# SonyCSLParis/audio-metrics

Hardware: AMD Instinct MI355X
Metric: evaluate() embeddings/sec (FAD+KD+PRDC), 2×100k CLAP-512 sets, 1/2/4/8 GPUs (higher is better)
Workload: dtype f32

## Files before the change

### audio-metrics_amd/_lib.py

```python
import ctypes
import os
from ctypes import c_char_p, c_double, c_int, c_int64, c_size_t, c_void_p

from ._build import DEV_LIB_PATH, LIB_PATH

_P = c_void_p

SIGNATURES = {
    "am_version": (c_char_p, []),
    "am_status_string": (c_char_p, [c_int]),
    "am_last_error": (c_char_p, []),
    "am_stats_workspace_bytes": (c_size_t, [c_int64, c_int]),
    "am_stats_f32": (c_int, [_P, c_int64, c_int, c_int64, _P, _P, _P, c_size_t, _P]),
    "am_colsum_f32": (c_int, [_P, c_int64, c_int, c_int64, _P, _P, c_size_t, _P]),
    "am_scatter_f32": (c_int, [_P, c_int64, c_int, c_int64, _P, _P, _P, c_size_t, _P]),
    "am_stats_f64_workspace_bytes": (c_size_t, [c_int64, c_int]),
    "am_stats_f64": (c_int, [_P, c_int64, c_int, c_int64, _P, _P, _P, c_size_t, _P]),
    "am_colsum_f64": (c_int, [_P, c_int64, c_int, c_int64, _P, _P, c_size_t, _P]),
    "am_scatter_f64": (c_int, [_P, c_int64, c_int, c_int64, _P, _P, _P, c_size_t, _P]),
    "am_stats_gather_workspace_bytes": (c_size_t, [c_int64, c_int, c_int]),
    "am_stats_gather_f32": (c_int, [_P, c_int64, c_int64, c_int, _P, _P, c_int, _P, _P, _P, c_size_t, _P]),
    "am_stats_gather_f64": (c_int, [_P, c_int64, c_int64, c_int, _P, _P, c_int, _P, _P, _P, c_size_t, _P]),
    "am_stats_merge_f64": (c_int, [c_int64, _P, _P, c_int64, _P, _P, c_int, _P, _P, _P]),
    "am_stats_push_max_rows": (c_int, []),
    "am_stats_push_f32": (c_int, [_P, c_int64, c_int, c_int64, c_int64, _P, _P, _P, _P, c_int64, _P]),
    "am_frechet_workspace_bytes": (c_size_t, [c_int]),
    "am_frechet_f64": (c_int, [_P, _P, _P, _P, c_int, c_int, c_double, _P, _P, c_size_t, _P]),
    "am_frechet_first_block": (c_int, []),
    "am_frechet_enqueue_f64": (c_int, [_P, _P, _P, _P, c_int, c_int, c_int, c_int, c_double, _P, _P, c_size_t, _P]),
    "am_frechet_batch_workspace_bytes": (c_size_t, [c_int, c_int]),
    "am_frechet_batch_f64": (c_int, [_P, _P, _P, _P, c_int64, c_int, c_int, c_int, c_double, _P, _P, c_size_t, _P]),
    "am_frechet_groups_max_rows": (c_int, []),
    "am_frechet_groups_workspace_bytes": (c_size_t, [c_int64, c_int, c_int]),
    "am_frechet_groups_f32": (c_int, [_P, c_int64, c_int64, c_int, _P, _P, c_int, _P, _P, _P, _P, c_size_t, _P]),
    "am_frechet_groups_f64": (c_int, [_P, c_int64, c_int64, c_int, _P, _P, c_int, _P, _P, _P, _P, c_size_t, _P]),
    "am_apa_f64": (c_double, [c_double, c_double, c_double]),
    "am_kd_workspace_bytes": (c_size_t, [c_int, c_int]),
    "am_kd_poly_workspace_bytes": (c_size_t, [c_int, c_int, c_int]),
    "am_kd_poly_f32": (c_int, [_P, c_int64, c_int64, _P, c_int64, c_int64, c_int, _P, _P, c_int, c_int,
                               c_double, c_double, c_int, _P, _P, c_size_t, _P]),
    "am_kd_draw_indices": (c_int, [ctypes.c_uint64, ctypes.c_uint64, ctypes.c_uint64, ctypes.c_uint64, c_int64, c_int64, c_int,
                                   c_int, _P, _P]),
    "am_kd_rbf_workspace_bytes": (c_size_t, [c_int, c_int]),
    "am_kd_rbf_f32": (c_int, [_P, c_int64, c_int64, _P, c_int64, c_int64, c_int, _P, _P, c_int, c_int, c_double, _P, _P,
                              c_size_t, _P]),
    "am_pairwise_select_workspace_bytes": (c_size_t, [c_int64, c_int]),
    "am_pairwise_select_f32": (c_int, [_P, c_int64, c_int64, c_int, c_int64, _P, _P, c_size_t, _P]),
    "am_mmd_rbf_workspace_bytes": (c_size_t, [c_int64, c_int64, c_int, ctypes.c_uint]),
# ... 120 lines not shown
```

### audio-metrics_amd/csrc/evaluate.hip

```cpp
#include "am_common.h"
#include <algorithm>
#include <vector>

namespace am {

__global__ void eval_pack_kernel(const double* __restrict__ fad5, const long long* __restrict__ totals, double* __restrict__ out,
                                 unsigned what) {
    const int t = threadIdx.x;
    if (t < AM_EVAL_HEAD) {
        double v = 0.0;
        if (t < 5) v = (what & AM_EVAL_FAD) ? fad5[t] : (t == 4 ? -1.0 : 0.0);
        else if (t < 9) v = (what & AM_EVAL_PRDC) ? (double)totals[t - 5] : 0.0;
        out[t] = v;
    }
}

struct EvalLayout {
    size_t total = 0;
    size_t stats_ws = 0, knn_ws = 0, prdc_ws = 0, kd_ws = 0, fad_ws = 0;
    double *mean[2] = {nullptr, nullptr}, *cov[2] = {nullptr, nullptr};
    float *norms[2] = {nullptr, nullptr}, *radii[2] = {nullptr, nullptr};
    uint32_t* pstats[2] = {nullptr, nullptr};
    uint16_t* half[2] = {nullptr, nullptr};
    int32_t* col = nullptr;
// ... 52 lines not shown
    return L.total;
}

extern "C" int am_evaluate_f32(const float* ref, int64_t n_ref, int64_t ld_ref, const float* cand, int64_t n_cand,
                               int64_t ld_cand, int D, unsigned what, int nearest_k, const int64_t* idx_cand,
                               const int64_t* idx_ref, int kd_subsets, int kd_m, double kd_gamma, double kd_coef0, int kd_degree,
                               const am_evaluate_side* given_ref, const am_evaluate_side* given_cand, double* out, void* ws,
                               size_t ws_bytes, am_stream_t stream, am_stream_t side_stream) {
    AM_REQUIRE(ref && cand && out, AM_ERR_BAD_ARG, "null pointer");
    AM_REQUIRE(n_ref >= 1 && n_cand >= 1 && D >= 1, AM_ERR_BAD_SHAPE, "sets of %lld and %lld rows x %d", (long long)n_ref,
               (long long)n_cand, D);
    AM_REQUIRE((what & ~(unsigned)(AM_EVAL_FAD | AM_EVAL_KD | AM_EVAL_PRDC)) == 0 && what != 0, AM_ERR_BAD_ARG, "what = %u", what);
    AM_REQUIRE(!(what & AM_EVAL_KD) || (idx_cand && idx_ref && kd_subsets >= 1 && kd_m >= 1), AM_ERR_BAD_ARG,
               "kernel distance needs the two index tables");
    AM_REQUIRE(!(what & AM_EVAL_FAD) || side_stream != stream, AM_ERR_BAD_ARG,
               "the Frechet solve runs on side_stream, which must differ from stream");
    hipStream_t st = static_cast<hipStream_t>(stream), side = static_cast<hipStream_t>(side_stream);
#ifdef AM_DEV_KNOBS
    static const int fad_place = getenv("AM_EVAL_FAD_PLACE") ? atoi(getenv("AM_EVAL_FAD_PLACE")) : 0;
#else
    constexpr int fad_place = 0;
#endif
    Carver c(ws, ws_bytes);
    EvalLayout L;
    AM_REQUIRE(eval_layout(c, n_ref, n_cand, D, nearest_k, kd_subsets, kd_m, what, L), AM_ERR_WORKSPACE,
               "workspace too small: need %zu bytes, have %zu", L.total, ws_bytes);
    const float* X[2] = {ref, cand};
    const int64_t n[2] = {n_ref, n_cand}, ld[2] = {ld_ref, ld_cand};
    const am_evaluate_side* given[2] = {given_ref, given_cand};
    int rc;

    const double* mean[2];
    const double* cov[2];
    if (what & AM_EVAL_FAD) {
        for (int s = 0; s < 2; ++s) {
            if (given[s] && given[s]->mean && given[s]->cov) {
                mean[s] = given[s]->mean;
                cov[s] = given[s]->cov;
                continue;
            }
            double* m_out = given[s] && given[s]->mean_out ? given[s]->mean_out : L.mean[s];
            double* c_out = given[s] && given[s]->cov_out ? given[s]->cov_out : L.cov[s];
            if ((rc = am_stats_f32(X[s], n[s], D, ld[s], m_out, c_out, L.ws_main, L.ws_main_bytes, stream)) != AM_OK) return rc;
            mean[s] = m_out;
            cov[s] = c_out;
        }
    }
    struct EventGuard {
        hipEvent_t e = nullptr;
        ~EventGuard() {
            if (e) (void)hipEventDestroy(e);
        }
    } ev_stats, ev_fad;
    if ((what & AM_EVAL_FAD) && fad_place != 2) {
        AM_HIP_TRY(hipEventCreateWithFlags(&ev_stats.e, hipEventDisableTiming));
        AM_HIP_TRY(hipEventRecord(ev_stats.e, st));
    }

    if (what & AM_EVAL_PRDC) {
        am_prepared_set prep[2];
        for (int s = 0; s < 2; ++s) {
            if ((rc = am_prepare_set_f32(X[s], n[s], ld[s], D, L.norms[s], L.pstats[s], L.half[s], stream)) != AM_OK) return rc;
            prep[s].norms = L.norms[s];
            prep[s].stats = L.pstats[s];
            prep[s].half = L.half[s];
        }
        const float* radii[2];
        for (int s = 0; s < 2; ++s) {
            if (given[s] && given[s]->radii) {
                radii[s] = given[s]->radii;
                continue;
            }
            float* r_out = given[s] && given[s]->radii_out ? given[s]->radii_out : L.radii[s];
            if ((rc = am_knn_radii_prepared_f32(X[s], n[s], ld[s], D, &prep[s], nearest_k, r_out, L.ws_main, L.ws_main_bytes,
                                                stream)) != AM_OK)
                return rc;
            radii[s] = r_out;
            if ((what & AM_EVAL_FAD) && fad_place == 2 && ev_stats.e == nullptr) {
                AM_HIP_TRY(hipEventCreateWithFlags(&ev_stats.e, hipEventDisableTiming));
                AM_HIP_TRY(hipEventRecord(ev_stats.e, st));
            }
        }
        if ((rc = am_prdc_counts_prepared_f32(ref, n_ref, ld_ref, &prep[0], cand, n_cand, ld_cand, &prep[1], D, radii[0], radii[1],
                                              L.col, L.rany, L.rcov, nullptr, L.ws_main, L.ws_main_bytes, stream)) != AM_OK)
            return rc;
        if ((rc = am_prdc_reduce(L.col, n_cand, L.rany, L.rcov, n_ref, reinterpret_cast<int64_t*>(L.totals), stream)) != AM_OK)
            return rc;
    }

    if (what & AM_EVAL_KD) {
        if ((rc = am_kd_poly_f32(cand, n_cand, ld_cand, ref, n_ref, ld_ref, D, idx_cand, idx_ref, kd_subsets, kd_m, kd_gamma,
                                 kd_coef0, kd_degree, out + AM_EVAL_HEAD, L.ws_main, L.ws_main_bytes, stream)) != AM_OK)
            return rc;
    }

// ... 378 lines not shown
```

### audio-metrics_amd/csrc/pairwise.hip

```cpp
#include "pairwise_common.h"
#include <algorithm>
#include <vector>
#include <cmath>
#include <type_traits>

namespace am {

__global__ void __launch_bounds__(256) row_sqnorm_kernel(const float* __restrict__ X, int64_t N, int64_t ld,
                                                         int D, float* __restrict__ out) {
    const int lane = threadIdx.x & 63;
    const int64_t row = (int64_t)blockIdx.x * 4 + (threadIdx.x >> 6);
    if (row >= N) return;
    const float* x = X + row * ld;
    float acc = 0.f;
    for (int k = lane * 4; k < D; k += 256) {
        const f32x4 v = load_k4(x, k, D);
        acc = fmaf(v.x, v.x, acc);
        acc = fmaf(v.y, v.y, acc);
        acc = fmaf(v.z, v.z, acc);
        acc = fmaf(v.w, v.w, acc);
    }
#pragma unroll
    for (int off = 32; off >= 1; off >>= 1) acc = acc + __shfl_xor(acc, off);
    if (lane == 0) out[row] = acc;
// ... 1226 lines not shown
    L.total = c.off;
    return c.ok();
}
size_t prdc64_filter_workspace(int64_t Nr, int64_t Nc, int D) {
    Carver c(nullptr, 0);
    Prdc64Layout L;
    prdc64_layout(c, Nr, Nc, D, L);
    return L.total;
}

int prdc64_filter(const double* R, int64_t Nr, int64_t ldr, const double* C, int64_t Nc, int64_t ldc, int D, const double* rt,
                  const double* ct, int32_t* col_count, unsigned* row_any, unsigned* row_cover, const int** fail_flag, void* ws,
                  size_t ws_bytes, hipStream_t st) {
    Carver c(ws, ws_bytes);
    Prdc64Layout L;
    AM_REQUIRE(prdc64_layout(c, Nr, Nc, D, L), AM_ERR_WORKSPACE, "workspace too small: need %zu bytes, have %zu", L.total, ws_bytes);
    hipLaunchKernelGGL(cast64_kernel, dim3((unsigned)ceil_div(Nr * L.ld32, 256)), dim3(256), 0, st, R, Nr, ldr, D, L.r32, L.ld32);
    hipLaunchKernelGGL(cast64_kernel, dim3((unsigned)ceil_div(Nc * L.ld32, 256)), dim3(256), 0, st, C, Nc, ldc, D, L.c32, L.ld32);
    hipLaunchKernelGGL(narrow64_kernel, dim3((unsigned)ceil_div(Nr, 256)), dim3(256), 0, st, rt, Nr, L.rt);
    hipLaunchKernelGGL(narrow64_kernel, dim3((unsigned)ceil_div(Nc, 256)), dim3(256), 0, st, ct, Nc, L.ct);
    hipLaunchKernelGGL(fill_u32_kernel, dim3((unsigned)ceil_div(Nr, 256)), dim3(256), 0, st, L.rmin, Nr, 0x7f800000u);
    AM_LAUNCH_CHECK();
    int rc;
    if ((rc = norms_of(nullptr, L.r32, Nr, L.ld32, D, L.rn, st)) != AM_OK) return rc;
    if ((rc = norms_of(nullptr, L.c32, Nc, L.ld32, D, L.cn, st)) != AM_OK) return rc;
    const Prdc64Hook h{R, C, ldr, ldc, rt, ct};
    if ((rc = run_cross_fast(L.r32, Nr, L.ld32, L.rn, L.rt, L.c32, Nc, L.ld32, L.cn, L.ct, D, L.plan, L.buf, col_count, L.rmin, row_any,
                             row_cover, false, st, nullptr, nullptr, &h)) != AM_OK)
        return rc;
    *fail_flag = L.buf.ov_count + 1;
    return AM_OK;
}

}

extern "C" int am_knn_radii_f32(const float* X, int64_t N, int64_t ldx, const float* Y, int64_t M, int64_t ldy,
                                int D, int k, float* out_r, void* ws, size_t ws_bytes, am_stream_t stream) {
    return knn_radii_impl(X, N, ldx, Y, M, ldy, D, k, out_r, ws, ws_bytes, stream, nullptr);
}

static bool prepared_ok(const am_prepared_set* p) { return p != nullptr && p->norms != nullptr && p->stats != nullptr && p->half != nullptr; }
static PreparedSet prepared_of(const am_prepared_set* p) { return PreparedSet{p->norms, p->stats, p->half}; }

extern "C" int64_t am_prepared_half_ld(int D) { return D < 1 ? 0 : half_ld(D); }

extern "C" int am_prepare_set_f32(const float* X, int64_t N, int64_t ld, int D, float* norms, uint32_t* stats4, uint16_t* half,
                                  am_stream_t stream) {
    int rc;
    if ((rc = check_matrix(X, N, ld, D, "X")) != AM_OK) return rc;
    AM_REQUIRE(norms && stats4 && half, AM_ERR_BAD_ARG, "null output pointer");
    hipStream_t st = static_cast<hipStream_t>(stream);
    if ((rc = launch_norms(X, N, ld, D, norms, st)) != AM_OK) return rc;
    AM_HIP_TRY(hipMemsetAsync(stats4, 0, 4 * sizeof(unsigned), st));
    return launch_to_half(X, N, ld, D, norms, stats4, 0, half, st);
}

extern "C" int am_knn_radii_prepared_f32(const float* X, int64_t N, int64_t ldx, int D, const am_prepared_set* prepared, int k,
                                         float* out_r, void* ws, size_t ws_bytes, am_stream_t stream) {
    AM_REQUIRE(prepared_ok(prepared), AM_ERR_BAD_ARG, "prepared set has a null member");
    const PreparedSet ps = prepared_of(prepared);
    return knn_radii_impl(X, N, ldx, X, N, ldx, D, k, out_r, ws, ws_bytes, stream, &ps);
}

extern "C" int am_filter_stats_enable(int64_t* device_slots) {
    if (device_slots == nullptr) {
        g_filter_stats = nullptr;
// ... 354 lines not shown
```

### audio-metrics_amd/csrc/pairwise_common.h

```cpp
#pragma once
#include "am_common.h"
#include "tile_engine.h"
#include <stdlib.h>

namespace am {

constexpr int EV_DEFAULT = EV_RSRC | EV_FRAGDB | EV_EARLY;
constexpr int WIDE_TILE_ROWS = 256;

#ifdef AM_DEV_KNOBS
static int env_int(const char* name, int dflt) {
    const char* v = getenv(name);
    return v ? atoi(v) : dflt;
}
static int engine_variant() {
    static const int v = env_int("AM_ENGINE_VARIANT", EV_DEFAULT);
    return v;
}
#else
static constexpr int env_int(const char*, int dflt) { return dflt; }
static constexpr int engine_variant() { return EV_DEFAULT; }
#endif

struct WorkItem {
    int64_t prow0;
    int64_t qtile0;
    int ntiles;
};

__device__ __forceinline__ WorkItem work_item(int64_t q_tiles, int nchunks, int order = 0) {
    int chunk = blockIdx.x % nchunks;
    int64_t rb = blockIdx.x / nchunks;
    if (order == 1) {
        const int64_t nrb = gridDim.x / nchunks;
        chunk = (int)(blockIdx.x / nrb);
        rb = blockIdx.x % nrb;
    }
    WorkItem w;
    w.prow0 = rb * TB;
    w.qtile0 = q_tiles * chunk / nchunks;
    w.ntiles = (int)(q_tiles * (chunk + 1) / nchunks - w.qtile0);
    return w;
}

static inline int choose_chunks(int64_t p_rows, int64_t q_rows) {
    const int64_t row_blocks = ceil_div(p_rows, TB);
    const int64_t q_tiles = ceil_div(q_rows, TB);
    static const int target = env_int("AM_WG_TARGET", 8192);
    int64_t want = ceil_div(target, row_blocks);
    if (want < 8) want = 8;
    want = ceil_div(want, 8) * 8;
    if (want > q_tiles) want = q_tiles;
    if (want > 64) want = 64;
    return (int)(want < 1 ? 1 : want);
}

static inline int check_matrix(const float* p, int64_t n, int64_t ld, int D, const char* name) {
    AM_REQUIRE(p != nullptr, AM_ERR_BAD_ARG, "%s is null", name);
    AM_REQUIRE(n >= 1 && D >= 1, AM_ERR_BAD_SHAPE, "%s has shape %lld x %d", name, (long long)n, D);
    AM_REQUIRE(aligned16(p) && ld % 4 == 0 && ld >= D, AM_ERR_BAD_ARG,
               "%s must be 16-byte aligned with ld %% 4 == 0 and ld >= D (ld=%lld, D=%d)", name, (long long)ld, D);
    return AM_OK;
}

__device__ __forceinline__ float sqrt_rn(float x) { return (float)sqrt((double)x); }

__global__ void row_sqnorm_kernel(const float* __restrict__ X, int64_t N, int64_t ld, int D, float* __restrict__ out);
int launch_norms(const float* X, int64_t N, int64_t ld, int D, float* out, hipStream_t st);


__device__ __forceinline__ int half_scale_exp(unsigned maxabs_bits) {
    if (maxabs_bits == 0u) return 0;
    const int e = (int)((maxabs_bits >> 23) & 255u) - 127;
    const int ex = 13 - e;
    return ex < -60 ? -60 : (ex > 60 ? 60 : ex);
}
__device__ __forceinline__ bool half_scale_ok(unsigned maxabs_bits) {
    if (maxabs_bits == 0u) return true;
    const int e = (int)((maxabs_bits >> 23) & 255u) - 127;
    return e != 128 && e != -127 && 13 - e >= -60 && 13 - e <= 60;
}
__device__ __forceinline__ float half_unscale(unsigned maxabs_bits_x, unsigned maxabs_bits_y) {
    const int s = half_scale_exp(maxabs_bits_x) + half_scale_exp(maxabs_bits_y);
    return -2.f * __uint_as_float((unsigned)(127 - s) << 23);
}


struct SymWork {
    int W;
    int64_t pb;
    int64_t qa;
    int ntiles;
};

__host__ __device__ __forceinline__ SymWork sym_item(int64_t T, int win_tiles, int W, int64_t pb, int part, int nparts) {
    const int64_t q0 = (int64_t)W * win_tiles;
    const int64_t q1 = (q0 + win_tiles < T) ? q0 + win_tiles : T;
    int64_t noff = T / 2 + 1;
    if ((T % 2) == 0 && pb >= T / 2) noff = T / 2;
    int64_t qa = pb > q0 ? pb : q0, qb = (pb + noff < q1) ? pb + noff : q1;
    if (qa >= qb) {
        qa = q0;
        qb = (pb + noff - T < q1) ? pb + noff - T : q1;
    }
    const int ntiles = qb > qa ? (int)(qb - qa) : 0;
    SymWork w;
    w.W = W;
    w.pb = pb;
    w.qa = qa;
    w.ntiles = (ntiles == 0 || (int)(pb * nparts / T) != part) ? 0 : ntiles;
    return w;
}

// ... 302 lines not shown
```

### audio-metrics_amd/csrc/pairwise_fast.h

```cpp
#pragma once

namespace am {

constexpr int EV_FAST = EV_DEFAULT | EV_F16 | EV_LDS;
constexpr int FAST_MAX_DIM = 4096;
constexpr int FAST_MIN_DIM = 1;
constexpr int FAST_DROP_BITS = 0;
static inline int half_drop_bits() {
    static const int n = std::min(std::max(env_int("AM_HALF_DROP_BITS", FAST_DROP_BITS), 0), 6);
    return n;
}
static inline float fast_c(int D) {
    const int n = half_drop_bits();
    const float rest = 1.9073486328125e-06f + 2.98023223876953125e-08f * sqrtf((float)D) + (float)(D + 1) * 4.76837158203125e-07f;
    if (n == 0) return 0.0009765625f + rest;
    const float u = ldexpf(1.f, -(11 - n)) + ldexpf(1.f, -11);
    return 2.f * u + u * u + rest;
}
constexpr int FAST_LDH_ALIGN = 64;

static inline int64_t half_ld(int D) { return (int64_t)(D + FAST_LDH_ALIGN - 1) / FAST_LDH_ALIGN * FAST_LDH_ALIGN; }

__global__ void __launch_bounds__(256) maxabs_bits_kernel(const float* __restrict__ X, int64_t N, int64_t ld, int D,
                                                          unsigned* __restrict__ out) {
    const int lane = threadIdx.x & 63;
    unsigned m = 0u;
    for (int64_t row = (int64_t)blockIdx.x * 4 + (threadIdx.x >> 6); row < N; row += (int64_t)gridDim.x * 4) {
        const float* x = X + row * ld;
        for (int k = lane * 4; k < D; k += 256) {
            const f32x4 v = load_k4(x, k, D);
            m = max(max(m, __float_as_uint(v.x) & 0x7fffffffu), __float_as_uint(v.y) & 0x7fffffffu);
            m = max(max(m, __float_as_uint(v.z) & 0x7fffffffu), __float_as_uint(v.w) & 0x7fffffffu);
        }
    }
#pragma unroll
    for (int off = 32; off >= 1; off >>= 1) m = max(m, (unsigned)__shfl_xor((int)m, off));
    __shared__ unsigned wave_max[4];
    if (lane == 0) wave_max[threadIdx.x >> 6] = m;
    __syncthreads();
    if (threadIdx.x == 0) {
        m = max(max(wave_max[0], wave_max[1]), max(wave_max[2], wave_max[3]));
        if (m != 0u) atomicMax(out, m);
    }
}

__global__ void __launch_bounds__(256) to_half_kernel(const float* __restrict__ X, int64_t N, int64_t ld, int D, int64_t ldh,
                                                      const unsigned* __restrict__ maxabs_bits, uint16_t* __restrict__ Xh, int drop) {
    const int64_t per_row = ldh / 8;
    const int64_t idx = (int64_t)blockIdx.x * 256 + threadIdx.x;
    const int64_t row = idx / per_row;
    if (row >= N) return;
    const float sc = __uint_as_float((unsigned)(127 + half_scale_exp(*maxabs_bits)) << 23);
    const int c = (int)(idx % per_row) * 8;
    const f32x4 a = load_k4(X + row * ld, c, D), b = load_k4(X + row * ld, c + 4, D);
    auto h = [&](float v) {
        unsigned b = (unsigned)__builtin_bit_cast(unsigned short, (_Float16)(v * sc));
        if (drop > 0) {
            const unsigned mag = b & 0x7fffu;
            b = (b & 0x8000u) | ((mag + (1u << (drop - 1)) - 1u + ((mag >> drop) & 1u)) & ~((1u << drop) - 1u));
        }
        return b;
    };
    uint4 o;
    o.x = h(a.x) | (h(a.y) << 16);
    o.y = h(a.z) | (h(a.w) << 16);
    o.z = h(b.x) | (h(b.y) << 16);
    o.w = h(b.z) | (h(b.w) << 16);
    *reinterpret_cast<uint4*>(Xh + row * ldh + c) = o;
}

__global__ void __launch_bounds__(256) max_bits_kernel(const float* __restrict__ v, int64_t n, unsigned* __restrict__ out) {
    unsigned m = 0u;
    for (int64_t i = (int64_t)blockIdx.x * 256 + threadIdx.x; i < n; i += (int64_t)gridDim.x * 256)
        m = max(m, __float_as_uint(v[i]));
#pragma unroll
    for (int off = 32; off >= 1; off >>= 1) m = max(m, (unsigned)__shfl_xor((int)m, off));
    if ((threadIdx.x & 63) == 0 && m != 0u) atomicMax(out, m);
}

constexpr int FILTER_STATS_SLOTS = 16;
static long long* g_filter_stats = nullptr;
static int g_filter_stats_device = -1;

static long long* filter_stats_for_current_device() {
    if (g_filter_stats == nullptr) return nullptr;
    int dev = -1;
    if (hipGetDevice(&dev) != hipSuccess || dev != g_filter_stats_device) return nullptr;
    return g_filter_stats;
}

__global__ void __launch_bounds__(256) filter_stats_kernel(const int* __restrict__ wgq_count, int64_t nwg, long long* __restrict__ stats,
                                                           int slot_calls, int slot_queued, const unsigned long long* spill64,
                                                           const int* spill32, int spill_cap, int slot_spill, const int* extra_a,
                                                           int slot_a, const int* extra_b, int slot_b) {
    long long q = 0;
// ... 1492 lines not shown
```

### audio-metrics_amd/csrc/stats.hip

```cpp
#include "am_common.h"
#include "tile_engine.h"
#include <algorithm>

namespace am {

constexpr int SC_ROWS = 32;
constexpr int SC_LD = 128;
constexpr int SC_SLAB = SC_ROWS * SC_LD;
constexpr int SC_FLUSH = 8;

__global__ void __launch_bounds__(256) colsum_partial_kernel(const float* __restrict__ X, int64_t N, int64_t ld,
                                                             int D, int64_t rows_per_block,
                                                             double* __restrict__ partial) {
    __shared__ double red[256 * 4];
    const int tid = threadIdx.x;
    const int cgs = (D + 3) / 4;
    const int cpp = cgs < 256 ? cgs : 256;
    const int rpar = 256 / cpp;
    const int my_cg = tid % cpp, my_r = tid / cpp;
    const int64_t r0 = (int64_t)blockIdx.x * rows_per_block;
    const int64_t r1 = (r0 + rows_per_block < N) ? r0 + rows_per_block : N;
    for (int cg0 = 0; cg0 < cgs; cg0 += cpp) {
        const int cg = cg0 + my_cg;
        double s0 = 0, s1 = 0, s2 = 0, s3 = 0;
        if (cg < cgs && my_r < rpar) {
            int64_t row = r0 + my_r;
            for (; row + 3 * rpar < r1; row += 4 * rpar) {
                f32x4 v[4];
#pragma unroll
                for (int u = 0; u < 4; ++u) v[u] = load_k4(X + (row + u * rpar) * ld, cg * 4, D);
#pragma unroll
                for (int u = 0; u < 4; ++u) { s0 += (double)v[u].x; s1 += (double)v[u].y; s2 += (double)v[u].z; s3 += (double)v[u].w; }
            }
            for (; row < r1; row += rpar) {
                const f32x4 v = load_k4(X + row * ld, cg * 4, D);
                s0 += (double)v.x; s1 += (double)v.y; s2 += (double)v.z; s3 += (double)v.w;
            }
        }
        red[tid * 4 + 0] = s0; red[tid * 4 + 1] = s1; red[tid * 4 + 2] = s2; red[tid * 4 + 3] = s3;
        __syncthreads();
        if (my_r == 0 && cg < cgs) {
            for (int rr = 1; rr < rpar; ++rr) {
                const int o = (rr * cpp + my_cg) * 4;
                s0 += red[o]; s1 += red[o + 1]; s2 += red[o + 2]; s3 += red[o + 3];
            }
            double* out = partial + (int64_t)blockIdx.x * D + cg * 4;
            out[0] = s0;
            if (cg * 4 + 1 < D) out[1] = s1;
            if (cg * 4 + 2 < D) out[2] = s2;
            if (cg * 4 + 3 < D) out[3] = s3;
        }
        __syncthreads();
    }
}

constexpr int CSR_COLS = 16, CSR_PARTS = 16;
__global__ void __launch_bounds__(256) colsum_reduce_kernel(const double* __restrict__ partial, int nblocks, int D,
                                                            double scale, double* __restrict__ out) {
    __shared__ double red[CSR_PARTS][CSR_COLS];
    const int c = threadIdx.x % CSR_COLS, part = threadIdx.x / CSR_COLS;
    const int d = blockIdx.x * CSR_COLS + c;
    double s = 0;
    if (d < D) {
        int b = part;
        for (; b + 7 * CSR_PARTS < nblocks; b += 8 * CSR_PARTS) {
            double v[8];
#pragma unroll
            for (int u = 0; u < 8; ++u) v[u] = partial[(int64_t)(b + u * CSR_PARTS) * D + d];
#pragma unroll
            for (int u = 0; u < 8; ++u) s += v[u];
        }
        for (; b < nblocks; b += CSR_PARTS) s += partial[(int64_t)b * D + d];
    }
    red[part][c] = s;
    __syncthreads();
    if (part == 0 && d < D) {
        double t = red[0][c];
        for (int q = 1; q < CSR_PARTS; ++q) t += red[q][c];
        out[d] = t * scale;
    }
}

__device__ __forceinline__ void tri_decode(int t, int T, int& tp, int& tq) {
    tp = 0;
    int rem = t;
    while (rem >= T - tp) { rem -= T - tp; ++tp; }
    tq = tp + rem;
}
// ... 412 lines not shown
                              void* ws, size_t ws_bytes, am_stream_t stream) {
    int rc;
    if ((rc = check_x(X, N, D, ld)) != AM_OK) return rc;
    AM_REQUIRE(mean && scatter, AM_ERR_BAD_ARG, "mean/scatter is null");
    const StatsPlan p = plan_stats(N, D);
    Carver c(ws, ws_bytes);
    c.take<double>((size_t)p.cs_blocks * D);
    double* sc_part = c.take<double>((size_t)p.nslabs * p.ntri * TB * TB);
    AM_REQUIRE(c.ok(), AM_ERR_WORKSPACE, "workspace too small: need %zu bytes, have %zu", c.off, ws_bytes);
    return run_scatter(X, N, D, ld, mean, 1.0, scatter, sc_part, p, static_cast<hipStream_t>(stream));
}

extern "C" int am_stats_f32(const float* X, int64_t N, int D, int64_t ld, double* mean, double* cov, void* ws,
                            size_t ws_bytes, am_stream_t stream) {
    int rc;
    if ((rc = check_x(X, N, D, ld)) != AM_OK) return rc;
    AM_REQUIRE(mean && cov, AM_ERR_BAD_ARG, "mean/cov is null");
    hipStream_t st = static_cast<hipStream_t>(stream);
    const StatsPlan p = plan_stats(N, D);
    Carver c(ws, ws_bytes);
    double* cs_part = c.take<double>((size_t)p.cs_blocks * D);
    double* sc_part = c.take<double>((size_t)p.nslabs * p.ntri * TB * TB);
    AM_REQUIRE(c.ok(), AM_ERR_WORKSPACE, "workspace too small: need %zu bytes, have %zu", c.off, ws_bytes);
    if ((rc = run_colsum(X, N, D, ld, 1.0 / (double)N, mean, cs_part, p, st)) != AM_OK) return rc;
    if (N == 1) {
        hipLaunchKernelGGL(zero_f64_kernel, dim3((unsigned)ceil_div((int64_t)D * D, 256)), dim3(256), 0, st, cov,
                           (int64_t)D * D);
        AM_LAUNCH_CHECK();
        return AM_OK;
    }
    return run_scatter(X, N, D, ld, mean, 1.0 / (double)(N - 1), cov, sc_part, p, st);
}

extern "C" size_t am_stats_f64_workspace_bytes(int64_t N, int D) {
    if (N < 1 || D < 1) return 0;
    return stats64_ws(D, plan_stats64(N, D));
}

static int check_x64(const double* X, int64_t N, int D, int64_t ld) {
    AM_REQUIRE(X != nullptr, AM_ERR_BAD_ARG, "X is null");
    AM_REQUIRE(N >= 1 && D >= 1, AM_ERR_BAD_SHAPE, "X has shape %lld x %d", (long long)N, D);
    AM_REQUIRE(D <= 8192, AM_ERR_BAD_SHAPE, "float64 statistics take rows of up to 8192 elements (D=%d)", D);
    AM_REQUIRE(ld >= D, AM_ERR_BAD_ARG, "ld=%lld < D=%d", (long long)ld, D);
    return AM_OK;
}

static int run_colsum64(const double* X, int64_t N, int D, int64_t ld, double scale, double* out, double* cs_part, const Stats64Plan& p,
                        hipStream_t st) {
    hipLaunchKernelGGL(colsum64_partial_kernel, dim3(p.cs_blocks), dim3(256), 0, st, X, N, ld, D, p.cs_rows, cs_part);
    AM_LAUNCH_CHECK();
    hipLaunchKernelGGL(colsum_reduce_kernel, dim3((unsigned)ceil_div(D, CSR_COLS)), dim3(256), 0, st, cs_part, p.cs_blocks, D, scale, out);
    AM_LAUNCH_CHECK();
    return AM_OK;
}

static int run_scatter64(const double* X, int64_t N, int D, int64_t ld, const double* mean, double scale, double* out, double* sc_part,
                         const Stats64Plan& p, hipStream_t st) {
    hipLaunchKernelGGL(scatter64_partial_kernel, dim3((unsigned)(p.ntri * p.nslabs)), dim3(256), 0, st, X, N, ld, D, mean, p.slab_rows,
                       p.ntri, sc_part);
    AM_LAUNCH_CHECK();
    hipLaunchKernelGGL(scatter64_reduce_kernel, dim3(S64_TILE * S64_TILE / 256, (unsigned)p.ntri), dim3(256), 0, st, sc_part,
                       p.nslabs, p.ntri, D, scale, out);
    AM_LAUNCH_CHECK();
    return AM_OK;
}

// ... 76 lines not shown
```

### audio-metrics_amd/distributed.py

```python
import numpy as np
import torch
import torch.distributed as dist

from .metrics.kd import subset_indices, KID_SUBSETS, KID_SUBSET_SIZE, KID_DEGREE, KID_COEF0


def _plain_upload(array, dev):
    return torch.as_tensor(np.ascontiguousarray(array))


def _world(group):
    if dist.is_available() and dist.is_initialized():
        return dist.get_world_size(group), dist.get_rank(group)
    return 1, 0


COLLECTIVES_AT_WORLD_ONE = False
LAST_C_ENTRY_COLLECTIVES = None


def _alone(world):
    if world == 1 and COLLECTIVES_AT_WORLD_ONE and dist.is_available() and dist.is_initialized():
        return False
    return world == 1
# ... 312 lines not shown
        with _Exchange("knn_lists", "all_gather", lists, world):
            _all_gather_into(all_lists.view(-1), lists.view(-1), world, group)
        r_full = ops.knn_lists_finish(all_lists, full, k)
        return r_full[lo:hi], r_full
    if after_first_exchange is not None:
        after_first_exchange()
    if not _alone(world) and full.dtype == torch.float64 and hasattr(ops, "knn_path") and ops.knn_path(n, n, d, k) == 3 and k <= 10:
        r_full = ops.knn_radii(full, k)
        return r_full[lo:hi], r_full
    if _alone(world) and prepared is not None:
        r_local = ops.knn_radii(full, k, prepared=prepared)
    elif local.shape[0] > 0:
        r_local = ops.knn_radii(local, k, columns=full)
    else:
        r_local = torch.empty(0, dtype=torch.float64 if full.dtype == torch.float64 else torch.float32, device=full.device)
    return r_local, _all_gather_rows(r_local, counts, world, group, "radii")


def result_from_record(head, mmds, metrics, n_ref, n_cand, nearest_k):
    result = {}
    if "fad" in metrics:
        result["fad"] = head[0]
    if "kd" in metrics:
        result["kernel_distance_mean"] = float(np.mean(mmds))
        result["kernel_distance_std"] = float(np.std(mmds))
    if "prdc" in metrics:
        n_prec, n_rec, sum_cnt, n_cov = (int(v) for v in head[5:9])
        result.update(precision=n_prec / n_cand, recall=n_rec / n_ref,
                      density=(1.0 / float(nearest_k)) * (sum_cnt / n_cand), coverage=n_cov / n_ref)
    return result


def evaluate_single(ref, cand, metrics, nearest_k, ops, kid_subsets=KID_SUBSETS, kid_subset_size=KID_SUBSET_SIZE, rng_seed=1234,
                    given_ref=None, given_cand=None):
    from .metrics.kd import device_subset_indices
    n_ref, n_cand = ref.shape[0], cand.shape[0]
    if n_ref == 0 or n_cand == 0:
        raise ValueError(f"empty embedding set: {n_ref} reference and {n_cand} candidate rows over 1 ranks")
    if "fad" in metrics:
        from .metrics.fad import warn_if_rank_deficient
        warn_if_rank_deficient(n_ref, n_cand, ref.shape[1], ref.dtype)
    idx1 = idx2 = None
    if "kd" in metrics:
        m = kid_subset_size
        if m >= min(n_ref, n_cand):
            m = max(1, min(n_ref, n_cand) // 2)
        idx1, idx2 = device_subset_indices(n_cand, n_ref, kid_subsets, m, rng_seed, ref.device)
    stats = None
    if "fad" in metrics:
        d = ref.shape[1]
        given_ref, given_cand = dict(given_ref or {}), dict(given_cand or {})
        stats = []
        for given in (given_cand, given_ref):
            if given.get("mean") is None or given.get("cov") is None:
                given.setdefault("mean_out", torch.empty(d, dtype=torch.float64, device=ref.device))
                given.setdefault("cov_out", torch.empty((d, d), dtype=torch.float64, device=ref.device))
                stats += [given["mean_out"], given["cov_out"]]
            else:
                stats += [given["mean"], given["cov"]]
    head, mmds = ops.evaluate(ref, cand, metrics, nearest_k, idx1, idx2, None, KID_COEF0, KID_DEGREE, given_ref, given_cand)
    if "fad" in metrics:
        code = int(head[4])
        if code == 4:
            from ._lib import HipLibraryError
            raise HipLibraryError("am_evaluate_f32: non-finite covariance product or trace in Newton-Schulz")
        if code == 0:
            head[0] = ops.frechet(*stats)["fd"]
    return result_from_record(head, mmds, metrics, n_ref, n_cand, nearest_k)


def _evaluate_sharded_c(ref_local, cand_local, ref_counts, cand_counts, metrics, nearest_k, group, ops, kid_subsets,
# ... 159 lines not shown
```

### audio-metrics_amd/hip_ops.py

```python
import ctypes
import os

import torch

from . import _lib


def _stream(device=None):
    return ctypes.c_void_p(torch.cuda.current_stream(device).cuda_stream)


def _ptr(t):
    return ctypes.c_void_p(t.data_ptr())


def _workspace(nbytes, device):
    return torch.empty(max(int(nbytes), 16), dtype=torch.uint8, device=device)


_SIDE_STREAMS = {}


def upload_host_array(array, device):
    import numpy as np
# ... 620 lines not shown
    check = _index_check(ws, idx, n, "group rows")
    return (out_groups, out_rows, check) if rows else (out_groups, check)


class PreparedSet:

    def __init__(self, norms, stats, half, ld_half, source):
        self.norms, self.stats, self.half, self.ld_half = norms, stats, half, ld_half
        self.source = source

    def matches(self, x):
        return self.source == (x.data_ptr(), x.shape[0], x.shape[1])

    def rows(self, lo, hi):
        return PreparedSet(self.norms[lo:hi], self.stats, self.half[lo * self.ld_half:hi * self.ld_half], self.ld_half,
                           (self.source[0] + 0, hi - lo, self.source[2]))

    def struct(self):
        return _lib.PreparedSetStruct(self.norms.data_ptr(), self.stats.data_ptr(), self.half.data_ptr())


def prepare(x):
    if is_f64(x):
        return None
    lib = _lib.load()
    x = as_matrix(x)
    n, d = x.shape
    ldh = int(lib.am_prepared_half_ld(d))
    norms = torch.empty(n, dtype=torch.float32, device=x.device)
    stats = torch.empty(4, dtype=torch.int32, device=x.device)
    half = torch.empty(n * ldh, dtype=torch.int16, device=x.device)
    _call(lib, "am_prepare_set_f32", x.device, _ptr(x), n, _ld(x), d, _ptr(norms), _ptr(stats), _ptr(half))
    return PreparedSet(norms, stats, half, ldh, (x.data_ptr(), n, d))


def knn_radii(x, k, columns=None, prepared=None):
    lib = _lib.load()
    if is_f64(x) or is_f64(columns):
        x = as_matrix64(x)
        y = x if columns is None else as_matrix64(columns, "columns")
        n, d = x.shape
        if y.shape[1] != d:
            raise ValueError("feature dimensions differ")
        out = torch.empty(n, dtype=torch.float64, device=x.device)
        nb = lib.am_knn_f64_workspace_bytes(n, y.shape[0], d, int(k))
        ws = _workspace(nb, x.device)
        _call(lib, "am_knn_radii_f64", x.device, _ptr(x), n, _ld64(x), _ptr(y), y.shape[0], _ld64(y), d, int(k), _ptr(out), _ptr(ws), nb)
        return out
    x = as_matrix(x)
    y = x if columns is None else as_matrix(columns, "columns")
    n, d = x.shape
    if y.shape[1] != d:
        raise ValueError("feature dimensions differ")
    out = torch.empty(n, dtype=torch.float32, device=x.device)
    nb = lib.am_knn_workspace_bytes(n, y.shape[0], d, int(k))
    ws = _workspace(nb, x.device)
    if prepared is not None and columns is None:
        ps = prepared.struct()
        _call(lib, "am_knn_radii_prepared_f32", x.device, _ptr(x), n, _ld(x), d, ctypes.byref(ps), int(k), _ptr(out), _ptr(ws), nb)
        return out
    _call(lib, "am_knn_radii_f32", x.device, _ptr(x), n, _ld(x), _ptr(y), y.shape[0], _ld(y), d, int(k), _ptr(out),
                                    _ptr(ws), nb)
    return out


KNN_SEARCH_MAX_K = 32
# ... 313 lines not shown
```

### include/audio_metrics_hip.h

```cpp
#ifndef AUDIO_METRICS_HIP_H
#define AUDIO_METRICS_HIP_H

#include <stddef.h>
#include <stdint.h>

#ifdef __cplusplus
extern "C" {
#endif

typedef void* am_stream_t;

typedef enum am_status {
    AM_OK = 0,
    AM_ERR_BAD_ARG = -1,
    AM_ERR_BAD_SHAPE = -2,
    AM_ERR_UNSUPPORTED_K = -3,
    AM_ERR_WORKSPACE = -4,
    AM_ERR_NO_CONVERGENCE = -5,
    AM_ERR_HIP = -6
} am_status;

#define AM_MAX_K 31

const char* am_version(void);
const char* am_status_string(int status);
const char* am_last_error(void);

size_t am_stats_workspace_bytes(int64_t N, int D);
int am_stats_f32(const float* X, int64_t N, int D, int64_t ld,
                 double* mean, double* cov,
                 void* ws, size_t ws_bytes, am_stream_t stream);
int am_colsum_f32(const float* X, int64_t N, int D, int64_t ld,
                  double* colsum, void* ws, size_t ws_bytes, am_stream_t stream);
int am_scatter_f32(const float* X, int64_t N, int D, int64_t ld, const double* mean,
                   double* scatter, void* ws, size_t ws_bytes, am_stream_t stream);
size_t am_stats_f64_workspace_bytes(int64_t N, int D);
int am_stats_f64(const double* X, int64_t N, int D, int64_t ld,
                 double* mean, double* cov,
                 void* ws, size_t ws_bytes, am_stream_t stream);
int am_colsum_f64(const double* X, int64_t N, int D, int64_t ld,
                  double* colsum, void* ws, size_t ws_bytes, am_stream_t stream);
int am_scatter_f64(const double* X, int64_t N, int D, int64_t ld, const double* mean,
                   double* scatter, void* ws, size_t ws_bytes, am_stream_t stream);
size_t am_stats_gather_workspace_bytes(int64_t n_total, int B, int D);
int am_stats_gather_f32(const float* X, int64_t N, int64_t ld, int D,
                        const int64_t* idx, const int64_t* offsets, int B,
                        double* means, double* covs,
                        void* ws, size_t ws_bytes, am_stream_t stream);
int am_stats_gather_f64(const double* X, int64_t N, int64_t ld, int D,
                        const int64_t* idx, const int64_t* offsets, int B,
                        double* means, double* covs,
                        void* ws, size_t ws_bytes, am_stream_t stream);

int am_stats_merge_f64(int64_t n1, const double* mean1, const double* cov1,
                       int64_t n2, const double* mean2, const double* cov2,
                       int D, double* out_mean, double* out_cov, am_stream_t stream);

int am_stats_push_max_rows(void);
int am_stats_push_f32(const float* E, int64_t b, int D, int64_t ld, int64_t n_old,
                      const double* mean_in, double* mean_out, double* cov,
                      float* rows_out, int64_t ld_out, am_stream_t stream);

size_t am_frechet_workspace_bytes(int D);
int am_frechet_f64(const double* mu_x, const double* cov_x,
                   const double* mu_y, const double* cov_y, int D,
                   int max_iter, double tol, double* out_host,
                   void* ws, size_t ws_bytes, am_stream_t stream);
int am_frechet_first_block(void);
// ... 190 lines not shown
```

Baseline: 8.817 million.

## Fuse column-sum, row norms and max-abs stats into one pass over each set

Adds a set_pass kernel that reads each embedding matrix once and produces the column-sum partials for the mean, per-row squared norms, and the max-abs/max-norm stats used for half-precision scaling. evaluate() uses this combined am_stats_prepare_f32 when both FAD and PRDC are requested, instead of separate stats and prepare passes that each read the f32 data. This is meant to cut redundant global-memory reads of the 100k×512 sets. In exchange the fused kernel holds more registers and double accumulators, and it adds a Python-side unfused fallback flag.

```diff
diff --git a/audio-metrics_amd/_lib.py b/audio-metrics_amd/_lib.py
--- a/audio-metrics_amd/_lib.py
+++ b/audio-metrics_amd/_lib.py
@@ -14,6 +14,7 @@
     "am_stats_f32": (c_int, [_P, c_int64, c_int, c_int64, _P, _P, _P, c_size_t, _P]),
     "am_colsum_f32": (c_int, [_P, c_int64, c_int, c_int64, _P, _P, c_size_t, _P]),
     "am_scatter_f32": (c_int, [_P, c_int64, c_int, c_int64, _P, _P, _P, c_size_t, _P]),
+    "am_stats_prepare_f32": (c_int, [_P, c_int64, c_int64, c_int, _P, _P, _P, _P, _P, _P, c_size_t, _P]),
     "am_stats_f64_workspace_bytes": (c_size_t, [c_int64, c_int]),
     "am_stats_f64": (c_int, [_P, c_int64, c_int, c_int64, _P, _P, _P, c_size_t, _P]),
     "am_colsum_f64": (c_int, [_P, c_int64, c_int, c_int64, _P, _P, c_size_t, _P]),
diff --git a/audio-metrics_amd/csrc/evaluate.hip b/audio-metrics_amd/csrc/evaluate.hip
--- a/audio-metrics_amd/csrc/evaluate.hip
+++ b/audio-metrics_amd/csrc/evaluate.hip
@@ -108,6 +108,7 @@
 
     const double* mean[2];
     const double* cov[2];
+    bool prepared[2] = {false, false};
     if (what & AM_EVAL_FAD) {
         for (int s = 0; s < 2; ++s) {
             if (given[s] && given[s]->mean && given[s]->cov) {
@@ -117,7 +118,14 @@
             }
             double* m_out = given[s] && given[s]->mean_out ? given[s]->mean_out : L.mean[s];
             double* c_out = given[s] && given[s]->cov_out ? given[s]->cov_out : L.cov[s];
-            if ((rc = am_stats_f32(X[s], n[s], D, ld[s], m_out, c_out, L.ws_main, L.ws_main_bytes, stream)) != AM_OK) return rc;
+            if (what & AM_EVAL_PRDC) {
+                if ((rc = am_stats_prepare_f32(X[s], n[s], ld[s], D, m_out, c_out, L.norms[s], L.pstats[s], L.half[s], L.ws_main,
+                                               L.ws_main_bytes, stream)) != AM_OK)
+                    return rc;
+                prepared[s] = true;
+            } else if ((rc = am_stats_f32(X[s], n[s], D, ld[s], m_out, c_out, L.ws_main, L.ws_main_bytes, stream)) != AM_OK) {
+                return rc;
+            }
             mean[s] = m_out;
             cov[s] = c_out;
         }
@@ -136,7 +144,8 @@
     if (what & AM_EVAL_PRDC) {
         am_prepared_set prep[2];
         for (int s = 0; s < 2; ++s) {
-            if ((rc = am_prepare_set_f32(X[s], n[s], ld[s], D, L.norms[s], L.pstats[s], L.half[s], stream)) != AM_OK) return rc;
+            if (!prepared[s] && (rc = am_prepare_set_f32(X[s], n[s], ld[s], D, L.norms[s], L.pstats[s], L.half[s], stream)) != AM_OK)
+                return rc;
             prep[s].norms = L.norms[s];
             prep[s].stats = L.pstats[s];
             prep[s].half = L.half[s];
diff --git a/audio-metrics_amd/csrc/pairwise.hip b/audio-metrics_amd/csrc/pairwise.hip
--- a/audio-metrics_amd/csrc/pairwise.hip
+++ b/audio-metrics_amd/csrc/pairwise.hip
@@ -1282,6 +1282,14 @@
     return AM_OK;
 }
 
+int launch_half_copy(const float* X, int64_t N, int64_t ld, int D, const unsigned* stats4, uint16_t* half, hipStream_t st) {
+    const int64_t ldh = half_ld(D);
+    hipLaunchKernelGGL(to_half_kernel, dim3((unsigned)ceil_div(N * (ldh / 8), 256)), dim3(256), 0, st, X, N, ld, D, ldh, stats4 + 2, half,
+                       half_drop_bits());
+    AM_LAUNCH_CHECK();
+    return AM_OK;
+}
+
 }
 
 extern "C" int am_knn_radii_f32(const float* X, int64_t N, int64_t ldx, const float* Y, int64_t M, int64_t ldy,
diff --git a/audio-metrics_amd/csrc/pairwise_common.h b/audio-metrics_amd/csrc/pairwise_common.h
--- a/audio-metrics_amd/csrc/pairwise_common.h
+++ b/audio-metrics_amd/csrc/pairwise_common.h
@@ -2,6 +2,7 @@
 #include "am_common.h"
 #include "tile_engine.h"
 #include <stdlib.h>
+#include <algorithm>
 
 namespace am {
 
@@ -63,10 +64,20 @@
     return AM_OK;
 }
 
+constexpr int FAST_DROP_BITS = 0;
+static inline int half_drop_bits() {
+    static const int n = std::min(std::max(env_int("AM_HALF_DROP_BITS", FAST_DROP_BITS), 0), 6);
+    return n;
+}
+constexpr int FAST_LDH_ALIGN = 64;
+
+static inline int64_t half_ld(int D) { return (int64_t)(D + FAST_LDH_ALIGN - 1) / FAST_LDH_ALIGN * FAST_LDH_ALIGN; }
+
 __device__ __forceinline__ float sqrt_rn(float x) { return (float)sqrt((double)x); }
 
 __global__ void row_sqnorm_kernel(const float* __restrict__ X, int64_t N, int64_t ld, int D, float* __restrict__ out);
 int launch_norms(const float* X, int64_t N, int64_t ld, int D, float* out, hipStream_t st);
+int launch_half_copy(const float* X, int64_t N, int64_t ld, int D, const unsigned* stats4, uint16_t* half, hipStream_t st);
 
 
 __device__ __forceinline__ int half_scale_exp(unsigned maxabs_bits) {
@@ -79,6 +90,17 @@
     if (maxabs_bits == 0u) return true;
     const int e = (int)((maxabs_bits >> 23) & 255u) - 127;
     return e != 128 && e != -127 && 13 - e >= -60 && 13 - e <= 60;
+}
+__device__ __forceinline__ float half_scale_factor(unsigned maxabs_bits) {
+    return __uint_as_float((unsigned)(127 + half_scale_exp(maxabs_bits)) << 23);
+}
+__device__ __forceinline__ unsigned half_image(float v, float sc, int drop) {
+    unsigned b = (unsigned)__builtin_bit_cast(unsigned short, (_Float16)(v * sc));
+    if (drop > 0) {
+        const unsigned mag = b & 0x7fffu;
+        b = (b & 0x8000u) | ((mag + (1u << (drop - 1)) - 1u + ((mag >> drop) & 1u)) & ~((1u << drop) - 1u));
+    }
+    return b;
 }
 __device__ __forceinline__ float half_unscale(unsigned maxabs_bits_x, unsigned maxabs_bits_y) {
     const int s = half_scale_exp(maxabs_bits_x) + half_scale_exp(maxabs_bits_y);
diff --git a/audio-metrics_amd/csrc/pairwise_fast.h b/audio-metrics_amd/csrc/pairwise_fast.h
--- a/audio-metrics_amd/csrc/pairwise_fast.h
+++ b/audio-metrics_amd/csrc/pairwise_fast.h
@@ -5,11 +5,6 @@
 constexpr int EV_FAST = EV_DEFAULT | EV_F16 | EV_LDS;
 constexpr int FAST_MAX_DIM = 4096;
 constexpr int FAST_MIN_DIM = 1;
-constexpr int FAST_DROP_BITS = 0;
-static inline int half_drop_bits() {
-    static const int n = std::min(std::max(env_int("AM_HALF_DROP_BITS", FAST_DROP_BITS), 0), 6);
-    return n;
-}
 static inline float fast_c(int D) {
     const int n = half_drop_bits();
     const float rest = 1.9073486328125e-06f + 2.98023223876953125e-08f * sqrtf((float)D) + (float)(D + 1) * 4.76837158203125e-07f;
@@ -17,10 +12,6 @@
     const float u = ldexpf(1.f, -(11 - n)) + ldexpf(1.f, -11);
     return 2.f * u + u * u + rest;
 }
-constexpr int FAST_LDH_ALIGN = 64;
-
-static inline int64_t half_ld(int D) { return (int64_t)(D + FAST_LDH_ALIGN - 1) / FAST_LDH_ALIGN * FAST_LDH_ALIGN; }
-
 __global__ void __launch_bounds__(256) maxabs_bits_kernel(const float* __restrict__ X, int64_t N, int64_t ld, int D,
                                                           unsigned* __restrict__ out) {
     const int lane = threadIdx.x & 63;
@@ -50,17 +41,10 @@
     const int64_t idx = (int64_t)blockIdx.x * 256 + threadIdx.x;
     const int64_t row = idx / per_row;
     if (row >= N) return;
-    const float sc = __uint_as_float((unsigned)(127 + half_scale_exp(*maxabs_bits)) << 23);
+    const float sc = half_scale_factor(*maxabs_bits);
     const int c = (int)(idx % per_row) * 8;
     const f32x4 a = load_k4(X + row * ld, c, D), b = load_k4(X + row * ld, c + 4, D);
-    auto h = [&](float v) {
-        unsigned b = (unsigned)__builtin_bit_cast(unsigned short, (_Float16)(v * sc));
-        if (drop > 0) {
-            const unsigned mag = b & 0x7fffu;
-            b = (b & 0x8000u) | ((mag + (1u << (drop - 1)) - 1u + ((mag >> drop) & 1u)) & ~((1u << drop) - 1u));
-        }
-        return b;
-    };
+    auto h = [&](float v) { return half_image(v, sc, drop); };
     uint4 o;
     o.x = h(a.x) | (h(a.y) << 16);
     o.y = h(a.z) | (h(a.w) << 16);
diff --git a/audio-metrics_amd/csrc/stats.hip b/audio-metrics_amd/csrc/stats.hip
--- a/audio-metrics_amd/csrc/stats.hip
+++ b/audio-metrics_amd/csrc/stats.hip
@@ -1,5 +1,6 @@
 #include "am_common.h"
 #include "tile_engine.h"
+#include "pairwise_common.h"
 #include <algorithm>
 
 namespace am {
@@ -54,6 +55,107 @@
     }
 }
 
+constexpr int SP_ROWS = 4;
+template <int TG>
+__global__ void __launch_bounds__(256) set_pass_kernel(const float* __restrict__ X, int64_t N, int64_t ld, int D,
+                                                       int64_t rows_per_block, double* __restrict__ partial,
+                                                       float* __restrict__ norms, unsigned* __restrict__ stats4) {
+    __shared__ double red[256 * 4];
+    __shared__ unsigned wave_max[2][4];
+    const int lane = threadIdx.x & 63, wave = threadIdx.x >> 6;
+    const int cgs = (D + 3) / 4;
+    const int rpar = 256 / cgs;
+    const int cols4 = cgs * 4;
+    const int64_t r0 = (int64_t)blockIdx.x * rows_per_block;
+    const int64_t r1 = (r0 + rows_per_block < N) ? r0 + rows_per_block : N;
+    unsigned mabs = 0u, mnorm = 0u;
+    f32x4 bufA[SP_ROWS][TG], bufB[SP_ROWS][TG];
+    auto issue = [&](f32x4 (&buf)[SP_ROWS][TG], int64_t row) {
+#pragma unroll
+        for (int u = 0; u < SP_ROWS; ++u) {
+            const int64_t rr = row + (int64_t)u * rpar;
+            if (rr < r1) {
+#pragma unroll
+                for (int t = 0; t < TG; ++t) buf[u][t] = load_k4(X + rr * ld, (lane + 64 * t) * 4, D);
+            }
+        }
+    };
+    for (int cls = wave; cls < rpar; cls += 4) {
+        double s[TG][4];
+#pragma unroll
+        for (int t = 0; t < TG; ++t) s[t][0] = s[t][1] = s[t][2] = s[t][3] = 0.0;
+        auto consume = [&](const f32x4 (&buf)[SP_ROWS][TG], int64_t row) {
+#pragma unroll
+            for (int u = 0; u < SP_ROWS; ++u) {
+                const int64_t rr = row + (int64_t)u * rpar;
+                if (rr >= r1) break;
+                float acc = 0.f;
+#pragma unroll
+                for (int t = 0; t < TG; ++t) {
+                    const f32x4 v = buf[u][t];
+                    s[t][0] += (double)v.x; s[t][1] += (double)v.y; s[t][2] += (double)v.z; s[t][3] += (double)v.w;
+                    if ((lane + 64 * t) * 4 < D) {
+                        acc = fmaf(v.x, v.x, acc);
+                        acc = fmaf(v.y, v.y, acc);
+                        acc = fmaf(v.z, v.z, acc);
+                        acc = fmaf(v.w, v.w, acc);
+                    }
+                    mabs = max(max(mabs, __float_as_uint(v.x) & 0x7fffffffu), __float_as_uint(v.y) & 0x7fffffffu);
+                    mabs = max(max(mabs, __float_as_uint(v.z) & 0x7fffffffu), __float_as_uint(v.w) & 0x7fffffffu);
+                }
+#pragma unroll
+                for (int off = 32; off >= 1; off >>= 1) acc = acc + __shfl_xor(acc, off);
+                if (lane == 0) {
+                    norms[rr] = acc;
+                    mnorm = max(mnorm, __float_as_uint(acc));
+                }
+            }
+        };
+        const int64_t step = (int64_t)SP_ROWS * rpar;
+        int64_t row = r0 + cls;
+        issue(bufA, row);
+        for (; row < r1; row += 2 * step) {
+            issue(bufB, row + step);
+            consume(bufA, row);
+            issue(bufA, row + 2 * step);
+            consume(bufB, row + step);
+        }
+#pragma unroll
+        for (int t = 0; t < TG; ++t) {
+            const int c = (lane + 64 * t) * 4;
+            if (c < cols4) {
+                double* r = red + cls * cols4 + c;
+                r[0] = s[t][0]; r[1] = s[t][1]; r[2] = s[t][2]; r[3] = s[t][3];
+            }
+        }
+    }
+    __syncthreads();
+    if ((int)threadIdx.x < cgs) {
+        const int c = threadIdx.x * 4;
+        double s0 = red[c], s1 = red[c + 1], s2 = red[c + 2], s3 = red[c + 3];
+        for (int rr = 1; rr < rpar; ++rr) {
+            const double* r = red + rr * cols4 + c;
+            s0 += r[0]; s1 += r[1]; s2 += r[2]; s3 += r[3];
+        }
+        double* out = partial + (int64_t)blockIdx.x * D + c;
+        out[0] = s0;
+        if (c + 1 < D) out[1] = s1;
+        if (c + 2 < D) out[2] = s2;
+        if (c + 3 < D) out[3] = s3;
+    }
+#pragma unroll
+    for (int off = 32; off >= 1; off >>= 1) mabs = max(mabs, (unsigned)__shfl_xor((int)mabs, off));
+    if (lane == 0) {
+        wave_max[0][wave] = mnorm;
+        wave_max[1][wave] = mabs;
+    }
+    __syncthreads();
+    if (threadIdx.x < 2) {
+        const unsigned m = max(max(wave_max[threadIdx.x][0], wave_max[threadIdx.x][1]), max(wave_max[threadIdx.x][2], wave_max[threadIdx.x][3]));
+        if (m != 0u) atomicMax(stats4 + 2 * threadIdx.x, m);
+    }
+}
+
 constexpr int CSR_COLS = 16, CSR_PARTS = 16;
 __global__ void __launch_bounds__(256) colsum_reduce_kernel(const double* __restrict__ partial, int nblocks, int D,
                                                             double scale, double* __restrict__ out) {
@@ -532,6 +634,36 @@
     return run_scatter(X, N, D, ld, mean, 1.0 / (double)(N - 1), cov, sc_part, p, st);
 }
 
+constexpr int SET_PASS_MAX_DIM = 1024;
+extern "C" int am_stats_prepare_f32(const float* X, int64_t N, int64_t ld, int D, double* mean, double* cov, float* norms,
+                                    uint32_t* stats4, uint16_t* half, void* ws, size_t ws_bytes, am_stream_t stream) {
+    int rc;
+    if ((rc = check_x(X, N, D, ld)) != AM_OK) return rc;
+    AM_REQUIRE(mean && cov && norms && stats4 && half, AM_ERR_BAD_ARG, "null output pointer");
+    AM_REQUIRE(aligned16(half), AM_ERR_BAD_ARG, "half must be 16-byte aligned");
+    hipStream_t st = static_cast<hipStream_t>(stream);
+    const StatsPlan p = plan_stats(N, D);
+    Carver c(ws, ws_bytes);
+    double* cs_part = c.take<double>((size_t)p.cs_blocks * D);
+    double* sc_part = c.take<double>((size_t)p.nslabs * p.ntri * TB * TB);
+    c.take<double>(D);
+    AM_REQUIRE(c.ok(), AM_ERR_WORKSPACE, "workspace too small: need %zu bytes (am_stats_workspace_bytes), have %zu", c.off, ws_bytes);
+    if (N == 1 || D > SET_PASS_MAX_DIM) {
+        if ((rc = am_stats_f32(X, N, D, ld, mean, cov, ws, ws_bytes, stream)) != AM_OK) return rc;
+        return am_prepare_set_f32(X, N, ld, D, norms, stats4, half, stream);
+    }
+    AM_HIP_TRY(hipMemsetAsync(stats4, 0, 4 * sizeof(unsigned), st));
+    const int tg = (int)ceil_div(ceil_div(D, 4), 64);
+    auto pass = tg <= 1 ? set_pass_kernel<1> : tg == 2 ? set_pass_kernel<2> : set_pass_kernel<4>;
+    hipLaunchKernelGGL(pass, dim3(p.cs_blocks), dim3(256), 0, st, X, N, ld, D, p.cs_rows, cs_part, norms, stats4);
+    AM_LAUNCH_CHECK();
+    hipLaunchKernelGGL(colsum_reduce_kernel, dim3((unsigned)ceil_div(D, CSR_COLS)), dim3(256), 0, st, cs_part, p.cs_blocks, D,
+                       1.0 / (double)N, mean);
+    AM_LAUNCH_CHECK();
+    if ((rc = launch_half_copy(X, N, ld, D, stats4, half, st)) != AM_OK) return rc;
+    return run_scatter(X, N, D, ld, mean, 1.0 / (double)(N - 1), cov, sc_part, p, st);
+}
+
 extern "C" size_t am_stats_f64_workspace_bytes(int64_t N, int D) {
     if (N < 1 || D < 1) return 0;
     return stats64_ws(D, plan_stats64(N, D));
diff --git a/audio-metrics_amd/distributed.py b/audio-metrics_amd/distributed.py
--- a/audio-metrics_amd/distributed.py
+++ b/audio-metrics_amd/distributed.py
@@ -368,11 +368,18 @@
 
 
 def evaluate_single(ref, cand, metrics, nearest_k, ops, kid_subsets=KID_SUBSETS, kid_subset_size=KID_SUBSET_SIZE, rng_seed=1234,
-                    given_ref=None, given_cand=None):
+                    given_ref=None, given_cand=None, fused=True):
     from .metrics.kd import device_subset_indices
     n_ref, n_cand = ref.shape[0], cand.shape[0]
     if n_ref == 0 or n_cand == 0:
         raise ValueError(f"empty embedding set: {n_ref} reference and {n_cand} candidate rows over 1 ranks")
+    if not fused:
+        given_ref, given_cand = dict(given_ref or {}), dict(given_cand or {})
+        for x, given in ((ref, given_ref), (cand, given_cand)):
+            if "fad" in metrics and (given.get("mean") is None or given.get("cov") is None):
+                given["mean"], given["cov"] = ops.stats(x)
+            if "prdc" in metrics and given.get("radii") is None:
+                given["radii"] = ops.knn_radii(x, nearest_k, prepared=ops.prepare(x))
     if "fad" in metrics:
         from .metrics.fad import warn_if_rank_deficient
         warn_if_rank_deficient(n_ref, n_cand, ref.shape[1], ref.dtype)
diff --git a/audio-metrics_amd/hip_ops.py b/audio-metrics_amd/hip_ops.py
--- a/audio-metrics_amd/hip_ops.py
+++ b/audio-metrics_amd/hip_ops.py
@@ -676,6 +676,26 @@
     half = torch.empty(n * ldh, dtype=torch.int16, device=x.device)
     _call(lib, "am_prepare_set_f32", x.device, _ptr(x), n, _ld(x), d, _ptr(norms), _ptr(stats), _ptr(half))
     return PreparedSet(norms, stats, half, ldh, (x.data_ptr(), n, d))
+
+
+def stats_prepare(x, ws=None):
+    lib = _lib.load()
+    x = as_matrix(x)
+    n, d = x.shape
+    ldh = int(lib.am_prepared_half_ld(d))
+    mean = torch.empty(d, dtype=torch.float64, device=x.device)
+    cov = torch.empty((d, d), dtype=torch.float64, device=x.device)
+    norms = torch.empty(n, dtype=torch.float32, device=x.device)
+    stats = torch.empty(4, dtype=torch.int32, device=x.device)
+    half = torch.empty(n * ldh, dtype=torch.int16, device=x.device)
+    nb = lib.am_stats_workspace_bytes(n, d)
+    if ws is None:
+        ws = _workspace(nb, x.device)
+    elif ws.numel() < nb:
+        raise ValueError(f"workspace of {ws.numel()} bytes, {nb} needed")
+    _call(lib, "am_stats_prepare_f32", x.device, _ptr(x), n, _ld(x), d, _ptr(mean), _ptr(cov), _ptr(norms), _ptr(stats), _ptr(half),
+          _ptr(ws), nb)
+    return mean, cov, PreparedSet(norms, stats, half, ldh, (x.data_ptr(), n, d))
 
 
 def knn_radii(x, k, columns=None, prepared=None):
diff --git a/include/audio_metrics_hip.h b/include/audio_metrics_hip.h
--- a/include/audio_metrics_hip.h
+++ b/include/audio_metrics_hip.h
@@ -34,6 +34,9 @@
                   double* colsum, void* ws, size_t ws_bytes, am_stream_t stream);
 int am_scatter_f32(const float* X, int64_t N, int D, int64_t ld, const double* mean,
                    double* scatter, void* ws, size_t ws_bytes, am_stream_t stream);
+int am_stats_prepare_f32(const float* X, int64_t N, int64_t ld, int D, double* mean, double* cov,
+                         float* norms, uint32_t* stats4, uint16_t* half,
+                         void* ws, size_t ws_bytes, am_stream_t stream);
 size_t am_stats_f64_workspace_bytes(int64_t N, int D);
 int am_stats_f64(const double* X, int64_t N, int D, int64_t ld,
                  double* mean, double* cov,
```

Result: no change. 8.828 million (median of 2 runs) (+0.1%).
